# HumaticsLAB/SEAM-Match-RCNN

Measured on AMD Instinct MI355X. Metric: video-clips/sec (10f x 800^2, 32 ROI/f, 1k gallery), higher is better.
Workload: dtype f32; 1 GPU; configs[1] full pipeline, fixed ROIs: 10 frames 800x800 -> ResNet-50-FPN + RPN head -> RoIAlign 14x14 (32 ROI/frame) -> mask head -> match trunk x2 -> SEAM NLB + attention pool (32 seq x 10) -> pair logits vs 1000-product bank -> top-20; hip_graph=False, hip_streams=2, frames=10, rois_per_frame=32, gallery=1000, topk=20, parallelism=single GPU

## Files before the change

include/seam_hip.h:

```cpp
#ifndef SEAM_HIP_H
#define SEAM_HIP_H

#include <stdint.h>

#ifdef __cplusplus
extern "C" {
#endif

typedef void* seam_stream_t;

int seam_version(void);
int seam_fastdiv_exact(unsigned d, unsigned long long n_max);
const char* seam_error_string(int code);

int seam_option_count(void);
const char* seam_option_name(int index);
int seam_set_option(const char* name, int value);
int seam_get_option(const char* name, int* value);

int seam_conv_kred(int C, int R, int S);
int seam_conv_rows_padded(int K);
int seam_conv_tile(int M, int K);
int seam_conv_tile_prec(int prec, int M, int K);
int seam_conv_tile_taps(int prec, int M, int K, int taps);
// ... 19 lines not shown

int seam_conv2d_dual_f32(const float* x1, const float* x2, const float* w_packed, const float* scale,
                         const float* shift, float* y, int N, int Ho, int Wo, int C1, int H2, int W2, int C2,
                         int stride2, int K, int relu, seam_stream_t stream);

int seam_conv1x1_sw_config(int M, int C1, int C2, int K);
int seam_conv1x1_sw_f32(const float* x, const float* x2, const float* w, const float* shift, const float* residual, float* y,
                        int M, int C1, int C2, int K, int relu, int res_mode, int Ho, int Wo, int rH, int rW,
                        seam_stream_t stream);

int seam_conv1x1_f16pc_supported(long long M, int C, int K);
long long seam_conv1x1_f16pc_weight_halves(int K, int C);
int seam_pack_conv1x1_weight_f16pc(const float* w, void* w_packed, int K, int C, seam_stream_t stream);
int seam_conv1x1_f16pc(const void* x, const void* w_packed, const float* scale, const float* shift, const void* residual, void* y,
                       long long M, int C, int K, int relu, seam_stream_t stream);

int seam_conv1x1_swh_config(long long M, int C1, int C2, int K);
int seam_conv1x1_swh_f16(const void* x, const void* x2, const void* w, const float* scale, const float* shift,
                         const void* residual, void* y, long long M, int C1, int C2, int K, int relu, int res_mode,
                         int Ho, int Wo, int rH, int rW, seam_stream_t stream);

int seam_stem_s2d_swh_f16(const void* xpad, const void* w, const float* scale, const float* shift, void* y, int N, int Ho, int Wo,
                          int relu, seam_stream_t stream);

int seam_conv1x1_pc_supported(long long M, int C, int K);
long long seam_conv1x1_pc_weight_floats(int K, int C);
int seam_pack_conv1x1_pc_f32(const float* w, float* w_packed, int K, int C, seam_stream_t stream);
int seam_conv1x1_pc_f32(const float* x, const float* w_packed, const float* scale, const float* shift, const float* residual,
                        float* y, long long M, int C, int K, int relu, seam_stream_t stream);

// ... 305 lines not shown
                             int64_t ws_bytes, const int64_t* scan, int* positions, int64_t capacity, int n, seam_stream_t stream);
int seam_rle_positions_paste(int D, int H, int W, const void* ws, int64_t ws_bytes, const int64_t* scan, int* positions,
                             int64_t capacity, seam_stream_t stream);

#define SEAM_SGD_MAX_SLOTS 32
#define SEAM_SGD_FP_SLOTS 64
typedef struct { float* p; const float* g; float* buf; int64_t numel; int group; int reserved; } seam_sgd_tensor_t;
typedef struct { int tensor; int count; int64_t offset; } seam_sgd_chunk_t;
typedef struct { float lr, momentum, one_minus_dampening, weight_decay; int nesterov, maximize, first, reserved; } seam_sgd_group_t;
typedef struct { int n; int reserved[3]; seam_sgd_group_t g[SEAM_SGD_MAX_SLOTS]; } seam_sgd_groups_t;
int seam_sgd_chunk_elems(void);
int seam_sgd_step_f32(const seam_sgd_tensor_t* tensors, const seam_sgd_chunk_t* chunks, int n_chunks,
                      const seam_sgd_groups_t* groups, unsigned long long* fingerprint, seam_stream_t stream);

enum { SEAM_REPACK_IGEMM = 0, SEAM_REPACK_WINO = 1, SEAM_REPACK_WINO24 = 2, SEAM_REPACK_PC = 3, SEAM_REPACK_SW = 4,
       SEAM_REPACK_SPLIT3 = 5, SEAM_REPACK_NARROW = 6 };
typedef struct {
    const float* src; void* dst; const float* scale;
    int64_t items;
    int form, K, Cin, R, S, Cstore, mode;
    int kred, rows, first_block, n_blocks, reserved;
} seam_repack_job_t;
long long seam_repack_layout(seam_repack_job_t* jobs, int n_jobs);
int seam_repack_many_f32(const seam_repack_job_t* jobs, int n_jobs, long long total_blocks, seam_stream_t stream);

#ifdef __cplusplus
}
#endif
#endif
```

seam-match-rcnn_amd/_native.py:

```python
from __future__ import annotations

import ctypes as C
import os

import torch

_HERE = os.path.dirname(os.path.abspath(__file__))
LIB_PATH = os.environ.get("SEAM_LIB_PATH") or os.path.join(_HERE, "lib", "libseam_hip.so")

_p = C.c_void_p
_i = C.c_int
_f = C.c_float
_i64 = C.c_int64

class TrunkLayer(C.Structure):
    _fields_ = [("w", C.c_void_p), ("u", C.c_void_p), ("u24", C.c_void_p), ("scale", C.c_void_p), ("shift", C.c_void_p)]


SGD_MAX_SLOTS = 32
SGD_FP_SLOTS = 64


class SgdTensor(C.Structure):
    _fields_ = [("p", C.c_void_p), ("g", C.c_void_p), ("buf", C.c_void_p), ("numel", C.c_int64), ("group", C.c_int), ("reserved", C.c_int)]


class SgdChunk(C.Structure):
    _fields_ = [("tensor", C.c_int), ("count", C.c_int), ("offset", C.c_int64)]


class SgdGroup(C.Structure):
    _fields_ = [("lr", C.c_float), ("momentum", C.c_float), ("one_minus_dampening", C.c_float), ("weight_decay", C.c_float),
                ("nesterov", C.c_int), ("maximize", C.c_int), ("first", C.c_int), ("reserved", C.c_int)]


class SgdGroups(C.Structure):
    _fields_ = [("n", C.c_int), ("reserved", C.c_int * 3), ("g", SgdGroup * SGD_MAX_SLOTS)]


REPACK_IGEMM, REPACK_WINO, REPACK_WINO24, REPACK_PC, REPACK_SW, REPACK_SPLIT3, REPACK_NARROW = range(7)


class RepackJob(C.Structure):
    _fields_ = [("src", C.c_void_p), ("dst", C.c_void_p), ("scale", C.c_void_p), ("items", C.c_int64),
                ("form", C.c_int), ("K", C.c_int), ("Cin", C.c_int), ("R", C.c_int), ("S", C.c_int), ("Cstore", C.c_int), ("mode", C.c_int),
                ("kred", C.c_int), ("rows", C.c_int), ("first_block", C.c_int), ("n_blocks", C.c_int), ("reserved", C.c_int)]


SIGNATURES = {
    "seam_version": (_i, []),
    "seam_fastdiv_exact": (_i, [C.c_uint, C.c_ulonglong]),
    "seam_error_string": (C.c_char_p, [_i]),
    "seam_option_count": (_i, []),
    "seam_option_name": (C.c_char_p, [_i]),
    "seam_set_option": (_i, [C.c_char_p, _i]),
# ... 13 lines not shown
    "seam_preprocess_s2d_batch_f32": (_i, [_p, C.c_size_t, _p, _i, _i, _i, _i, _i, _i, _i, _p]),
    "seam_preprocess_s2d_batch_f16": (_i, [_p, C.c_size_t, _p, _i, _i, _i, _i, _i, _i, _i, _p]),
    "seam_preprocess_s2d_pad_batch_f16": (_i, [_p, C.c_size_t, _p, _i, _i, _i, _i, _i, _i, _i, _i, _i, _p]),
    "seam_conv2d_dual_f32": (_i, [_p, _p, _p, _p, _p, _p, _i, _i, _i, _i, _i, _i, _i, _i, _i, _i, _p]),
    "seam_conv1x1_pc_supported": (_i, [C.c_longlong, _i, _i]),
    "seam_conv1x1_pc_weight_floats": (C.c_longlong, [_i, _i]),
    "seam_pack_conv1x1_pc_f32": (_i, [_p, _p, _i, _i, _p]),
    "seam_conv1x1_pc_f32": (_i, [_p, _p, _p, _p, _p, _p, C.c_longlong, _i, _i, _i, _p]),
    "seam_conv1x1_sw_config": (_i, [_i, _i, _i, _i]),
    "seam_conv1x1_sw_f32": (_i, [_p, _p, _p, _p, _p, _p, _i, _i, _i, _i, _i, _i, _i, _i, _i, _i, _p]),
    "seam_conv1x1_swh_config": (_i, [C.c_longlong, _i, _i, _i]),
    "seam_conv1x1_f16pc_supported": (_i, [C.c_longlong, _i, _i]),
    "seam_conv1x1_f16pc_weight_halves": (C.c_longlong, [_i, _i]),
    "seam_pack_conv1x1_weight_f16pc": (_i, [_p, _p, _i, _i, _p]),
    "seam_conv1x1_f16pc": (_i, [_p, _p, _p, _p, _p, _p, C.c_longlong, _i, _i, _i, _p]),
    "seam_conv1x1_swh_f16": (_i, [_p, _p, _p, _p, _p, _p, _p, C.c_longlong, _i, _i, _i, _i, _i, _i, _i, _i, _i, _p]),
    "seam_stem_s2d_swh_f16": (_i, [_p, _p, _p, _p, _p, _i, _i, _i, _i, _p]),
    "seam_conv2d_dual_f16": (_i, [_p, _p, _p, _p, _p, _p, _i, _i, _i, _i, _i, _i, _i, _i, _i, _i, _p]),
    "seam_conv2d_upres_f32": (_i, [_p, _p, _p, _p, _p, _p, _i, _i, _i, _i, _i, _i, _i, _i, _i, _i, _i, _i, _p]),
    "seam_pack_conv_weight_bx3": (_i, [_p, _p, _p, _i, _i, _i, _i, _i, _i, _p]),
    "seam_conv2d_bx3": (_i, [_p, _p, _p, _p, _p, _p, _i, _i, _i, _i, _i, _i, _i, _i, _i, _i, _p]),
    "seam_pack_conv_weight_sx": (_i, [_p, _p, _p, _i, _i, _i, _i, _i, _i, _p]),
    "seam_conv2d_sx": (_i, [_p, _p, _p, _p, _p, _p, _i, _i, _i, _i, _i, _i, _i, _i, _i, _i, _i, _p]),
    "seam_wino_supported": (_i, [_i, _i, _i, _i, _i]),
    "seam_wino_weight_floats": (C.c_longlong, [_i, _i]),
    "seam_wino_slot_fill_pct": (_i, [_i, _i, _i, _i, _i, _i]),
    "seam_wino_tile_variant": (_i, [_i, _i, _i, _i, _i, _i]),
    "seam_pack_conv_weight_wino_f32": (_i, [_p, _p, _i, _i, _i, _i, _p]),
    "seam_wino_issue_slots": (C.c_longlong, [_i, _i, _i, _i, _i, _i]),
    "seam_wino24_issue_slots": (C.c_longlong, [_i, _i, _i, _i, _i, _i]),
# ... 177 lines not shown
```

seam-match-rcnn_amd/csrc/seam_conv.hip:

```cpp
#include <hip/hip_runtime.h>
#include "seam_device.h"
#include "seam_launch.h"
#include <stdint.h>
#include <stdio.h>
#include <stdlib.h>
#include "seam_fastdiv.h"
#include "seam_fpn_common.h"
#include "seam_opts.h"
#include "seam_pack_items.h"

namespace {

constexpr int CHUNK_BYTES = 128;
constexpr int LDB = CHUNK_BYTES + 16;

struct ConvArgs {
    const void* x;
    const void* w;
    const float* scale;
    const float* shift;
    const void* res;
    void* y;
    int N, H, W, C;
    int Ho, Wo, K;
// ... 706 lines not shown
                eo[r] = (unsigned)(row * p.K + n);
            }
            if (p.res) {
#pragma unroll
                for (int r = 0; r < 16; ++r)
                    rv[r] = __builtin_bit_cast(float, __builtin_amdgcn_raw_buffer_load_b32(r_rsrc, nok ? eo[r] * 4u : kOob, 0, 0));
            }
#pragma unroll
            for (int r = 0; r < 16; ++r) {
                float v = acc[i][j][r] * sc + sh;
                if (p.res) v = p.relu == 2 ? (rv[r] > 0.f ? v : 0.f) : v + rv[r];
                if (p.relu == 1) v = fmaxf(v, 0.f);
                __builtin_amdgcn_raw_buffer_store_b32(__builtin_bit_cast(unsigned, v), y_rsrc, nok ? eo[r] * 4u : kOob, 0, 0);
            }
        }
    }
}

__device__ __forceinline__ float top16(float x) {
    unsigned t = __builtin_bit_cast(unsigned, x) & 0xffff0000u;
    asm volatile("" : "+v"(t));
    return __builtin_bit_cast(float, t);
}

__device__ __forceinline__ void split3_bf16(const f32x4 v, u32x2& p0, u32x2& p1, u32x2& p2) {
#pragma unroll
    for (int p = 0; p < 2; ++p) {
        const float a0 = top16(v[2 * p]), b0 = top16(v[2 * p + 1]);
        const float ra = v[2 * p] - a0, rb = v[2 * p + 1] - b0;
        const float a1 = top16(ra), b1 = top16(rb);
        const float sa = ra - a1, sb = rb - b1;
        p0[p] = (__builtin_bit_cast(unsigned, a0) >> 16) | __builtin_bit_cast(unsigned, b0);
        p1[p] = (__builtin_bit_cast(unsigned, a1) >> 16) | __builtin_bit_cast(unsigned, b1);
        p2[p] = (__builtin_bit_cast(unsigned, sa) >> 16) | (__builtin_bit_cast(unsigned, sb) & 0xffff0000u);
    }
}

template <int BM, int BN, int TERMS>
__global__ __launch_bounds__(256, BM * BN >= 128 * 128 ? 1 : 2) void conv_igemm_sx(const ConvArgs p) {
    static_assert(TERMS == 6 || TERMS == 9, "six or nine piece products");
    constexpr int NW = 4, ES = 4, EPV = 4, BKE = 32;
    constexpr int WM = BM / 2, WN = BN / 2;
    constexpr int MT = WM / 32, NT = WN / 32;
    constexpr int RP = 8 * NW;
    constexpr int AI = BM / RP;
    constexpr int VPP = BN * 4;
    constexpr int BI = 3 * VPP / 256;
    constexpr int Q = TERMS * MT * NT;
    constexpr int PA = BM * 64 + 64;
// ... 617 lines not shown
```

seam-match-rcnn_amd/csrc/seam_pack_items.h:

```cpp
#pragma once
#include <hip/hip_runtime.h>
#include <stddef.h>
#include "seam_device.h"

namespace seam_pack {

template <int BKE>
__device__ __forceinline__ float igemm_value(const float* __restrict__ w, size_t i, int K, int Cin, int R, int S, int Cstore, int nk,
                                             int bn, int mode) {
    const int col = (int)(i % BKE);
    size_t rest = i / BKE;
    const int row_in = (int)(rest % bn);
    rest /= bn;
    const int q = (int)(rest % nk);
    const int tn = (int)(rest / nk);
    const int row = tn * bn + row_in;
    int r, s2, c;
    if (Cstore >= BKE) {
        const int ccn = Cstore / BKE;
        s2 = q % S;
        c = ((q / S) % ccn) * BKE + col;
        r = q / (S * ccn);
    } else {
        const int kk = q * BKE + col;
// ... 105 lines not shown
        }
    }
}

__device__ __forceinline__ void pwpc_item(const float* __restrict__ w, float* __restrict__ out, size_t i, int C) {
    const int nsteps = C / 8;
    const int lane = (int)(i & 63);
    size_t rest = i >> 6;
    const int step = (int)(rest % nsteps); rest /= nsteps;
    const int nt = (int)rest;
    const int nn = nt * 32 + (lane & 31);
    const int c = 8 * step + 4 * (lane >> 5);
    *reinterpret_cast<f32x4*>(out + i * 4) = *reinterpret_cast<const f32x4*>(w + (size_t)nn * C + c);
}

__device__ __forceinline__ void narrow_item(const float* __restrict__ w, float* __restrict__ out, int i, int K, int C) {
    const int e = i & 3, lane = (i >> 2) & 63, j = i >> 8;
    const int col = lane & 15, kq = lane >> 4;
    out[i] = col < K ? w[(size_t)col * C + 16 * j + 4 * kq + e] : 0.f;
}

__device__ __forceinline__ void sw_item(const float* __restrict__ w, const float* __restrict__ scale, float* __restrict__ out, size_t i, int C) {
    const float v = w[i];
    out[i] = scale ? v * scale[i / (size_t)C] : v;
}

}
```

seam-match-rcnn_amd/csrc/seam_repack.hip:

```cpp
#include <hip/hip_runtime.h>
#include <stdint.h>
#include "seam_device.h"
#include "seam_hip.h"
#include "seam_pack_items.h"

namespace {

constexpr int JOB_BLOCKS = 512;

__global__ __launch_bounds__(256) void repack_many_kernel(const seam_repack_job_t* __restrict__ jobs, int n_jobs) {
    int lo = 0, hi = n_jobs;
    while (hi - lo > 1) {
        const int mid = lo + ((hi - lo) >> 1);
        if (jobs[mid].first_block <= (int)blockIdx.x) lo = mid; else hi = mid;
    }
    const seam_repack_job_t j = jobs[lo];
    const size_t i0 = (size_t)((int)blockIdx.x - j.first_block) * 256 + threadIdx.x;
    const size_t step = (size_t)j.n_blocks * 256;
    const size_t total = (size_t)j.items;
    const float* src = j.src;
    switch (j.form) {
    case SEAM_REPACK_IGEMM: {
        const int nk = j.kred / 32, bn = j.rows % 128 == 0 ? 128 : 64;
        float* out = (float*)j.dst;
// ... 4 lines not shown
        const int nk = j.kred / 32, bn = j.rows % 128 == 0 ? 128 : 64;
        unsigned short* out = (unsigned short*)j.dst;
        for (size_t i = i0; i < total; i += step)
            seam_pack::split3_item(seam_pack::igemm_value<32>(src, i, j.K, j.Cin, j.R, j.S, j.Cstore, nk, bn, j.mode), out, i, bn);
        break;
    }
    case SEAM_REPACK_WINO:
        for (size_t i = i0; i < total; i += step) seam_pack::wino_item(src, (float*)j.dst, i, j.K, j.Cin, j.Cstore / 8, j.mode);
        break;
    case SEAM_REPACK_WINO24:
        for (size_t i = i0; i < total; i += step) seam_pack::wino24_item(src, (float*)j.dst, i, j.K, j.Cin, j.Cstore / 8, j.mode);
        break;
    case SEAM_REPACK_PC:
        for (size_t i = i0; i < total; i += step) seam_pack::pwpc_item(src, (float*)j.dst, i, j.Cstore);
        break;
    case SEAM_REPACK_SW:
        for (size_t i = i0; i < total; i += step) seam_pack::sw_item(src, j.scale, (float*)j.dst, i, j.Cstore);
        break;
    case SEAM_REPACK_NARROW:
        for (size_t i = i0; i < total; i += step) seam_pack::narrow_item(src, (float*)j.dst, (int)i, j.K, j.Cstore);
        break;
    default:
        break;
    }
}

long long job_items(seam_repack_job_t& j) {
    if (!j.src || !j.dst || j.K < 1 || j.Cin < 1 || j.Cstore < j.Cin) return 0;
    const bool one = j.R == 1 && j.S == 1, plain = j.Cstore == j.Cin && j.mode == 0 && one;
    switch (j.form) {
// ... 2 lines not shown
        if (j.R < 1 || j.S < 1 || (j.Cstore % 4) || (j.Cstore >= 32 && j.Cstore % 32) || j.mode < 0 || j.mode > 2) return 0;
        if (j.mode == 1 && (!one || j.K % 4)) return 0;
        if ((long long)j.R * j.S * j.Cstore > (1 << 24)) return 0;
        j.kred = seam_conv_kred(j.Cstore, j.R, j.S);
        j.rows = seam_conv_rows_padded(j.K);
        return (long long)j.rows * j.kred;
    }
    case SEAM_REPACK_WINO:
    case SEAM_REPACK_WINO24:
        if (j.R != 3 || j.S != 3 || (j.mode != 0 && j.mode != 2) || !seam_wino_supported(j.Cstore, j.K, 3, 3, 1)) return 0;
        if ((j.K % 32) || (j.Cstore % 8)) return 0;
        return (long long)(j.K / 32) * (j.Cstore / 8) * 64;
    case SEAM_REPACK_PC:
        if (!plain || (j.K % 128) || (j.Cstore % 128) || (((uintptr_t)j.src | (uintptr_t)j.dst) & 15)) return 0;
        return (long long)j.K * j.Cstore / 4;
    case SEAM_REPACK_SW:
        if (!plain) return 0;
        return (long long)j.K * j.Cstore;
    case SEAM_REPACK_NARROW:
        if (!plain || !seam_linear_narrow_supported(j.Cstore, j.K)) return 0;
        return (long long)(j.Cstore >> 4) * 256;
    default:
        return 0;
    }
}

}

extern "C" {

// ... 28 lines not shown
```

seam-match-rcnn_amd/ops.py:

```python
from __future__ import annotations

import ctypes as C
from dataclasses import dataclass
from typing import Optional, Sequence

import torch

from . import _native

F32 = torch.float32
F16 = torch.float16


def _stream() -> int:
    return torch.cuda.current_stream().cuda_stream


def _req(t: torch.Tensor, dtype=F32, name: str = "tensor") -> torch.Tensor:
    if not isinstance(t, torch.Tensor) or not t.is_cuda:
        raise _native.SeamNativeError(f"{name}: expected a tensor on the HIP device (no CPU path exists)")
    if dtype is not None and t.dtype != dtype:
        raise TypeError(f"{name}: expected {dtype}, got {t.dtype}")
    return t if t.is_contiguous() else t.contiguous()

# ... 19 lines not shown
    R: int
    S: int
    stride: int = 1
    pad: int = 0
    Cin: int = 0
    dtype: object = F32
    u: Optional[torch.Tensor] = None
    u24: Optional[torch.Tensor] = None
    wn: Optional[torch.Tensor] = None
    ws: Optional[torch.Tensor] = None
    shift_sw: Optional[torch.Tensor] = None
    wq: Optional[torch.Tensor] = None
    wh: Optional[torch.Tensor] = None
    wsh: Optional[torch.Tensor] = None
    wph: Optional[torch.Tensor] = None


BX3 = "bf16x3"
SX6 = "bf16x6"
SX9 = "bf16x9"
_SX_TERMS = {SX6: 6, SX9: 9}


import os as _os
WINOGRAD = _os.environ.get("SEAM_WINOGRAD", "1") != "0"
F16PC = _os.environ.get("SEAM_F16PC", "1") != "0"
F16PC64 = _os.environ.get("SEAM_F16PC64", "1") != "0"
PWPC = _os.environ.get("SEAM_PWPC", "1") != "0"
SWH = _os.environ.get("SEAM_PWH", "1") != "0"
PWHPC = _os.environ.get("SEAM_PWHPC", "1") != "0"
PWHPC_MIN_C = int(_os.environ.get("SEAM_PWHPC_MIN_C", "1024"))
F16PC_RULE = True


def _pack_wino(lib, weight: torch.Tensor, K: int, cin: int, cs: int, mode: int) -> Optional[torch.Tensor]:
    if not lib.seam_wino_supported(cs, K, 3, 3, 1):
        return None
    u = torch.empty((int(lib.seam_wino_weight_floats(K, cs)),), dtype=F32, device=weight.device)
    _native.check(lib.seam_pack_conv_weight_wino_f32(_ptr(weight), _ptr(u), K, cin, cs, mode, _stream()),
                  "seam_pack_conv_weight_wino_f32")
    return u


def _pack_wino24(lib, weight: torch.Tensor, K: int, cin: int, cs: int, mode: int) -> Optional[torch.Tensor]:
    if not lib.seam_wino_supported(cs, K, 3, 3, 1):
        return None
# ... 70 lines not shown
    if transposed2x2:
        cin, cout = weight.shape[0], weight.shape[1]
        K, R, S, mode = 4 * cout, 1, 1, 1
    else:
        is_linear = weight.dim() == 2
        if weight.dim() == 2:
            weight = weight[:, :, None, None]
        if weight.dim() == 3:
            weight = weight[:, :, :, None]
        weight = weight.contiguous()
        K, cin, R, S = weight.shape
        mode = 0
    epv = 8 if dtype == F16 else 4
    cs = cstore if cstore is not None else ((cin + epv - 1) // epv) * epv
    rows = lib.seam_conv_rows_padded(K)
    u = u24 = wh = None
    if dtype == F32:
        kred = lib.seam_conv_kred(cs, R, S)
        wp = torch.empty((rows, kred), dtype=F32, device=weight.device)
        _native.check(lib.seam_pack_conv_weight_f32(_ptr(weight), _ptr(wp), K, cin, R, S, cs, mode, _stream()),
                      "seam_pack_conv_weight_f32")
        if wino and mode == 0 and R == 3 and S == 3 and stride == 1:
            u = _pack_wino(lib, weight, K, cin, cs, 0)
            u24 = _pack_wino24(lib, weight, K, cin, cs, 0) if u is not None else None
    elif dtype == BX3:
        kred = lib.seam_conv_kred(cs, R, S)
        wp = torch.empty((rows, kred), dtype=F32, device=weight.device)
        tmp = torch.empty((rows, kred), dtype=F32, device=weight.device)
        _native.check(lib.seam_pack_conv_weight_bx3(_ptr(weight), _ptr(wp), _ptr(tmp), K, cin, R, S, cs, mode, _stream()),
                      "seam_pack_conv_weight_bx3")
    elif dtype in _SX_TERMS:
        kred = lib.seam_conv_kred(cs, R, S)
        wp = torch.empty((rows, kred * 3), dtype=torch.bfloat16, device=weight.device)
        tmp = torch.empty((rows, kred), dtype=F32, device=weight.device)
        _native.check(lib.seam_pack_conv_weight_sx(_ptr(weight), _ptr(wp), _ptr(tmp), K, cin, R, S, cs, mode, _stream()),
                      "seam_pack_conv_weight_sx")
    else:
        kred = lib.seam_conv_kred_f16(cs, R, S)
        wp = torch.empty((rows, kred), dtype=F16, device=weight.device)
        _native.check(lib.seam_pack_conv_weight_f16(_ptr(weight), _ptr(wp), K, cin, R, S, cs, mode, _stream()),
                      "seam_pack_conv_weight_f16")
        if F16PC and mode == 0 and R == 3 and S == 3 and stride == 1 and pad in (0, 1) and ((cs % 128 == 0 and K % 128 == 0) or (cs == 64 and K == 64 and F16PC64)):
            wh = torch.empty((int(lib.seam_f16pc_weight_halves(K, cs)),), dtype=F16, device=weight.device)
            _native.check(lib.seam_pack_conv_weight_f16pc(_ptr(weight), _ptr(wh), K, cin, cs, _stream()), "seam_pack_conv_weight_f16pc")
    scale = shift = None
    if bias is not None:
        bias = bias.detach().to(F32)
        if transposed2x2:
            bias = bias.repeat(4)
    if bn is not None:
        bw, bb, rm, rv = (t.detach().to(F32) for t in bn)
# ... 20 lines not shown
            and lib.seam_conv1x1_pc_supported(1 << 20, cs, K)):
        wq = torch.empty((int(lib.seam_conv1x1_pc_weight_floats(K, cs)),), dtype=F32, device=weight.device)
        _native.check(lib.seam_pack_conv1x1_pc_f32(_ptr(weight.reshape(K, cin).to(F32).contiguous()), _ptr(wq), K, cs, _stream()),
                      "seam_pack_conv1x1_pc_f32")
    wsh = None
    if (SWH and dtype == F16 and mode in (0, 1) and not is_linear and R == 1 and S == 1 and stride == 1 and pad == 0 and cs == cin
            and lib.seam_conv1x1_swh_config(1 << 20, cs, 0, K)):
        wm = weight.permute(2, 3, 1, 0).reshape(K, cin) if transposed2x2 else weight.reshape(K, cin)
        wsh = wm.to(F16).contiguous()
    wph = None
    if (PWHPC and dtype == F16 and mode == 0 and not is_linear and R == 1 and S == 1 and stride == 1 and pad == 0 and cs == cin
            and lib.seam_conv1x1_f16pc_supported(1 << 20, cs, K)):
        wph = torch.empty((int(lib.seam_conv1x1_f16pc_weight_halves(K, cs)),), dtype=F16, device=weight.device)
        _native.check(lib.seam_pack_conv1x1_weight_f16pc(_ptr(weight.reshape(K, cin).to(F32).contiguous()), _ptr(wph), K, cs, _stream()),
                      "seam_pack_conv1x1_weight_f16pc")
    pc = PackedConv(wp, scale, shift, K, cs, R, S, stride, pad, cin, dtype, u, u24, wn, ws, shift_sw, wq, wh, wsh, wph)
    if _PACK_RECORDER is not None:
        _PACK_RECORDER.records.append((weight, bias, bn, mode, pc))
    return pc


def pack_conv_dgrad(weight: torch.Tensor, pad_fwd: int = 0, wino: bool = True) -> PackedConv:
    lib = _native.lib()
    weight = _req(weight.detach(), name="weight")
    if weight.dim() == 2:
        weight = weight[:, :, None, None]
    weight = weight.contiguous()
    cout, cin, R, S = weight.shape
    if cout % 32 or R != S:
        raise ValueError("pack_conv_dgrad: Cout must be a multiple of 32 and the kernel square")
    rows = lib.seam_conv_rows_padded(cin)
# ... 181 lines not shown
        e0, e1 = torch.cuda.Event(enable_timing=True), torch.cuda.Event(enable_timing=True)
        e0.record()
    lib = _native.lib()
    wino = pc.dtype == F32 and pc.u is not None and WINOGRAD and out_hw is None and _wino_pays(lib, n, h, w, c, pc.K, pc.pad)
    wino24 = wino and pc.u24 is not None and WINOGRAD24 and _wino24_pays(lib, n, h, w, c, pc.K, pc.pad)
    sw = not narrow and pc.dtype == F32 and out_hw is None and _sw_ok(pc, h, w)
    pwpc = (not narrow and not sw and pc.dtype == F32 and pc.wq is not None and PWPC and out_hw is None and h * w >= PWPC_MIN_HW
            and lib.seam_conv1x1_pc_supported(n * h * w, c, pc.K) == 1)
    f16pc = (pc.dtype == F16 and pc.wh is not None and F16PC and residual is None and out_hw is None and not out_f32 and relu in (0, 1, False, True)
             and (lib.seam_conv3x3_f16pc_pays if F16PC_RULE else lib.seam_conv3x3_f16pc_supported)(n, h, w, c, pc.K, pc.pad) == 1)
    pwhpc = (pc.dtype == F16 and pc.wph is not None and PWHPC and residual is None and out_hw is None and not out_f32
             and relu in (0, 1, False, True) and c >= PWHPC_MIN_C and h * w >= SW_MIN_HW
             and lib.seam_conv1x1_f16pc_supported(n * h * w, c, pc.K) == 1)
    swh = (not pwhpc and pc.dtype == F16 and pc.wsh is not None and SWH and out_hw is None and not out_f32 and h * w >= SW_MIN_HW
           and relu in (0, 1, False, True))
    if pwhpc:
        _native.check(lib.seam_conv1x1_f16pc(_ptr(x), _ptr(pc.wph), _ptr(pc.scale), _ptr(pc.shift), None, _ptr(y), n * h * w, c, pc.K,
                                             1 if relu else 0, _stream()), "seam_conv1x1_f16pc")
    elif swh:
        _native.check(lib.seam_conv1x1_swh_f16(_ptr(x), None, _ptr(pc.wsh), _ptr(pc.scale), _ptr(pc.shift), _ptr(residual), _ptr(y),
                                               n * h * w, c, 0, pc.K, 1 if relu else 0, 1 if residual is not None else 0, 0, 0, 0, 0,
                                               _stream()), "seam_conv1x1_swh_f16")
    elif narrow:
        _native.check(lib.seam_linear_narrow_f32(_ptr(x), _ptr(pc.wn), _ptr(pc.shift), _ptr(y), n * h * w, c, pc.K, int(relu), _stream()),
                      "seam_linear_narrow_f32")
    elif sw:
        _sw_launch(lib, x, None, pc, residual, y, n * h * w, c, 0, relu, 1 if residual is not None else 0)
    elif pwpc:
        _native.check(lib.seam_conv1x1_pc_f32(_ptr(x), _ptr(pc.wq), _ptr(pc.scale), _ptr(pc.shift), _ptr(residual), _ptr(y),
                                              n * h * w, c, pc.K, int(relu), _stream()), "seam_conv1x1_pc_f32")
    elif wino24:
# ... 17 lines not shown
    elif pc.dtype == BX3:
        _native.check(lib.seam_conv2d_bx3(_ptr(x), _ptr(pc.w), _ptr(pc.scale), _ptr(pc.shift), _ptr(residual), _ptr(y),
                                          n, h, w, c, pc.K, pc.R, pc.S, pc.stride, pc.pad, int(relu), _stream()),
                      "seam_conv2d_bx3")
    elif f16pc:
        _native.check(lib.seam_conv3x3_f16pc(_ptr(x), _ptr(pc.wh), _ptr(pc.scale), _ptr(pc.shift), None, _ptr(y),
                                             n, h, w, c, pc.K, pc.pad, 1 if relu else 0, _stream()), "seam_conv3x3_f16pc")
    else:
        _native.check(lib.seam_conv2d_f16(_ptr(x), _ptr(pc.w), _ptr(pc.scale), _ptr(pc.shift), _ptr(residual), _ptr(y),
                                          n, h, w, c, pc.K, pc.R, pc.S, pc.stride, pc.pad, 1 if relu else 0,
                                          1 if out_f32 else 0, _stream()), "seam_conv2d_f16")
    if trace is not None:
        e1.record()
        tile = lib.seam_conv_tile_taps(3 if pc.dtype in _SX_TERMS else 2 if pc.dtype == BX3 else 1 if pc.dtype == F16 else 0,
                                       n * ho * wo, pc.K, pc.R * pc.S)
        if pwhpc:
            variant = "conv1x1_f16pc"
        elif swh:
            variant = _swh_variant(lib, n * h * w, c, pc.K)
        elif narrow:
            variant = "linear_narrow"
        elif sw:
            variant = _sw_variant(lib, n * h * w, c, pc.K)
        elif pwpc:
            variant = "conv1x1_pc"
        elif wino24:
            variant = ("conv3x3_wino24pc" if lib.seam_wino24_form(n, h, w, c, pc.K, pc.pad) == 1
                       else f"conv3x3_wino24<{lib.seam_wino24_variant(n, h, w, c, pc.K, pc.pad)}>")
        elif wino:
            variant = f"conv3x3_wino<{lib.seam_wino_tile_variant(n, h, w, c, pc.K, pc.pad)}>"
        elif f16pc:
# ... 1382 lines not shown
                self._entries.append((wdeps, self._jobs_of(path, weight, mode, pc)))
            self._pk.append(pk)
            self._keys.append(m._pack_key())
        self.rebuilds += self._ever_built
        self._built = self._ever_built = True

    @staticmethod
    def _jobs_of(path, weight, mode, pc):
        N = _native

        def job(form, dst, R=1, S=1, cs=pc.Cstore, cin=pc.Cin, md=0, scale=None):
            return N.RepackJob(src=weight.data_ptr(), dst=dst.data_ptr(), scale=None if scale is None else scale.data_ptr(), form=form,
                               K=pc.K, Cin=cin, R=R, S=S, Cstore=cs, mode=md)

        if pc.dtype in _SX_TERMS:
            return [job(N.REPACK_SPLIT3, pc.w, pc.R, pc.S, md=mode)]
        if pc.dtype != F32 or pc.wh is not None or pc.wsh is not None or pc.wph is not None:
            raise NotImplementedError(f"PackPlan: {path}: only fp32 packs are refreshed in place (pass refresh_packs=False)")
        jobs = [job(N.REPACK_IGEMM, pc.w, pc.R, pc.S, md=mode)]
        if pc.u is not None:
            jobs.append(job(N.REPACK_WINO, pc.u, 3, 3, md=mode))
        if pc.u24 is not None:
            jobs.append(job(N.REPACK_WINO24, pc.u24, 3, 3, md=mode))
        if (pc.wn is not None or pc.ws is not None or pc.wq is not None) and mode != 0:
            raise NotImplementedError(f"PackPlan: {path}: the pointwise forms of a transposed conv are not covered")
        if pc.wn is not None:
            jobs.append(job(N.REPACK_NARROW, pc.wn))
        if pc.ws is not None and pc.ws.data_ptr() != weight.data_ptr():
            jobs.append(job(N.REPACK_SW, pc.ws, scale=pc.scale))
        if pc.wq is not None:
            jobs.append(job(N.REPACK_PC, pc.wq))
# ... 52 lines not shown
```

Before: 69.68 clips/s.

## Add warp-specialized persistent split-bf16 MFMA kernel for large SX6 1x1 convs

Adds a new persistent 1x1 convolution kernel for SX6 (bf16x3 split, six-term) packed layers. Producer waves load fp32 activations, split them into three bf16 planes in LDS, and double-buffer them. Consumer waves run 32x32x16 bf16 MFMAs against a pre-split weight pack streamed through a register ring, then apply a fused scale/shift/residual/relu epilogue. The kernel is used only when the tile count passes a threshold, and it adds a third weight pack per eligible layer plus a repack path. The aim is to replace the generic SX implicit-GEMM kernel for large pointwise convs with better overlap of loads and compute.

```diff
diff --git a/include/seam_hip.h b/include/seam_hip.h
--- a/include/seam_hip.h
+++ b/include/seam_hip.h
@@ -57,6 +57,12 @@
 int seam_pack_conv1x1_weight_f16pc(const float* w, void* w_packed, int K, int C, seam_stream_t stream);
 int seam_conv1x1_f16pc(const void* x, const void* w_packed, const float* scale, const float* shift, const void* residual, void* y,
                        long long M, int C, int K, int relu, seam_stream_t stream);
+
+int seam_conv1x1_sxpc_supported(long long M, int C, int K);
+long long seam_conv1x1_sxpc_weight_bytes(int K, int C);
+int seam_pack_conv1x1_weight_sxpc(const float* w, void* w_packed, int K, int C, seam_stream_t stream);
+int seam_conv1x1_sxpc(const float* x, const void* w_packed, const float* scale, const float* shift, const float* residual, float* y,
+                      long long M, int C, int K, int relu, seam_stream_t stream);
 
 int seam_conv1x1_swh_config(long long M, int C1, int C2, int K);
 int seam_conv1x1_swh_f16(const void* x, const void* x2, const void* w, const float* scale, const float* shift,
@@ -392,7 +398,7 @@
                       const seam_sgd_groups_t* groups, unsigned long long* fingerprint, seam_stream_t stream);
 
 enum { SEAM_REPACK_IGEMM = 0, SEAM_REPACK_WINO = 1, SEAM_REPACK_WINO24 = 2, SEAM_REPACK_PC = 3, SEAM_REPACK_SW = 4,
-       SEAM_REPACK_SPLIT3 = 5, SEAM_REPACK_NARROW = 6 };
+       SEAM_REPACK_SPLIT3 = 5, SEAM_REPACK_NARROW = 6, SEAM_REPACK_SXPC = 7 };
 typedef struct {
     const float* src; void* dst; const float* scale;
     int64_t items;
diff --git a/seam-match-rcnn_amd/_native.py b/seam-match-rcnn_amd/_native.py
--- a/seam-match-rcnn_amd/_native.py
+++ b/seam-match-rcnn_amd/_native.py
@@ -38,7 +38,7 @@
     _fields_ = [("n", C.c_int), ("reserved", C.c_int * 3), ("g", SgdGroup * SGD_MAX_SLOTS)]
 
 
-REPACK_IGEMM, REPACK_WINO, REPACK_WINO24, REPACK_PC, REPACK_SW, REPACK_SPLIT3, REPACK_NARROW = range(7)
+REPACK_IGEMM, REPACK_WINO, REPACK_WINO24, REPACK_PC, REPACK_SW, REPACK_SPLIT3, REPACK_NARROW, REPACK_SXPC = range(8)
 
 
 class RepackJob(C.Structure):
@@ -82,6 +82,10 @@
     "seam_conv1x1_f16pc_weight_halves": (C.c_longlong, [_i, _i]),
     "seam_pack_conv1x1_weight_f16pc": (_i, [_p, _p, _i, _i, _p]),
     "seam_conv1x1_f16pc": (_i, [_p, _p, _p, _p, _p, _p, C.c_longlong, _i, _i, _i, _p]),
+    "seam_conv1x1_sxpc_supported": (_i, [C.c_longlong, _i, _i]),
+    "seam_conv1x1_sxpc_weight_bytes": (C.c_longlong, [_i, _i]),
+    "seam_pack_conv1x1_weight_sxpc": (_i, [_p, _p, _i, _i, _p]),
+    "seam_conv1x1_sxpc": (_i, [_p, _p, _p, _p, _p, _p, C.c_longlong, _i, _i, _i, _p]),
     "seam_conv1x1_swh_f16": (_i, [_p, _p, _p, _p, _p, _p, _p, C.c_longlong, _i, _i, _i, _i, _i, _i, _i, _i, _i, _p]),
     "seam_stem_s2d_swh_f16": (_i, [_p, _p, _p, _p, _p, _i, _i, _i, _i, _p]),
     "seam_conv2d_dual_f16": (_i, [_p, _p, _p, _p, _p, _p, _i, _i, _i, _i, _i, _i, _i, _i, _i, _i, _p]),
diff --git a/seam-match-rcnn_amd/csrc/seam_conv.hip b/seam-match-rcnn_amd/csrc/seam_conv.hip
--- a/seam-match-rcnn_amd/csrc/seam_conv.hip
+++ b/seam-match-rcnn_amd/csrc/seam_conv.hip
@@ -744,25 +744,6 @@
                 __builtin_amdgcn_raw_buffer_store_b32(__builtin_bit_cast(unsigned, v), y_rsrc, nok ? eo[r] * 4u : kOob, 0, 0);
             }
         }
-    }
-}
-
-__device__ __forceinline__ float top16(float x) {
-    unsigned t = __builtin_bit_cast(unsigned, x) & 0xffff0000u;
-    asm volatile("" : "+v"(t));
-    return __builtin_bit_cast(float, t);
-}
-
-__device__ __forceinline__ void split3_bf16(const f32x4 v, u32x2& p0, u32x2& p1, u32x2& p2) {
-#pragma unroll
-    for (int p = 0; p < 2; ++p) {
-        const float a0 = top16(v[2 * p]), b0 = top16(v[2 * p + 1]);
-        const float ra = v[2 * p] - a0, rb = v[2 * p + 1] - b0;
-        const float a1 = top16(ra), b1 = top16(rb);
-        const float sa = ra - a1, sb = rb - b1;
-        p0[p] = (__builtin_bit_cast(unsigned, a0) >> 16) | __builtin_bit_cast(unsigned, b0);
-        p1[p] = (__builtin_bit_cast(unsigned, a1) >> 16) | __builtin_bit_cast(unsigned, b1);
-        p2[p] = (__builtin_bit_cast(unsigned, sa) >> 16) | (__builtin_bit_cast(unsigned, sb) & 0xffff0000u);
     }
 }
 
diff --git a/seam-match-rcnn_amd/csrc/seam_pack_items.h b/seam-match-rcnn_amd/csrc/seam_pack_items.h
--- a/seam-match-rcnn_amd/csrc/seam_pack_items.h
+++ b/seam-match-rcnn_amd/csrc/seam_pack_items.h
@@ -2,6 +2,7 @@
 #include <hip/hip_runtime.h>
 #include <stddef.h>
 #include "seam_device.h"
+#include "seam_split.h"
 
 namespace seam_pack {
 
@@ -143,6 +144,27 @@
     *reinterpret_cast<f32x4*>(out + i * 4) = *reinterpret_cast<const f32x4*>(w + (size_t)nn * C + c);
 }
 
+__device__ __forceinline__ void sxpc_item(const float* __restrict__ w, unsigned short* __restrict__ out, size_t i, int C) {
+    const int nsteps = C / 16;
+    const int lane = (int)(i & 63);
+    const size_t rest = i >> 6;
+    const int step = (int)(rest % nsteps);
+    const size_t nt = rest / nsteps;
+    const float* src = w + (nt * 32 + (lane & 31)) * (size_t)C + 16 * step + 8 * (lane >> 5);
+    unsigned short* o = out + (nt * nsteps + step) * 1536 + lane * 8;
+#pragma unroll
+    for (int e = 0; e < 8; ++e) {
+        const float x = src[e];
+        const float x0 = top16(x);
+        const float r = x - x0;
+        const float y0 = top16(r);
+        const float s = r - y0;
+        o[e] = (unsigned short)(__builtin_bit_cast(unsigned, x0) >> 16);
+        o[512 + e] = (unsigned short)(__builtin_bit_cast(unsigned, y0) >> 16);
+        o[1024 + e] = (unsigned short)(__builtin_bit_cast(unsigned, s) >> 16);
+    }
+}
+
 __device__ __forceinline__ void narrow_item(const float* __restrict__ w, float* __restrict__ out, int i, int K, int C) {
     const int e = i & 3, lane = (i >> 2) & 63, j = i >> 8;
     const int col = lane & 15, kq = lane >> 4;
diff --git a/seam-match-rcnn_amd/csrc/seam_pwsx.hip b/seam-match-rcnn_amd/csrc/seam_pwsx.hip
--- /dev/null
+++ b/seam-match-rcnn_amd/csrc/seam_pwsx.hip
@@ -0,0 +1,325 @@
+#include <hip/hip_runtime.h>
+#include "seam_device.h"
+#include <stdint.h>
+#include <type_traits>
+#include "seam_fastdiv.h"
+#include "seam_launch.h"
+#include "seam_pack_items.h"
+#include "seam_split.h"
+
+namespace {
+
+constexpr int BM = 128;
+constexpr int CK = 64;
+constexpr int KS = CK / 16;
+constexpr int PLB = CK * 2;
+constexpr int ROWB = 3 * PLB + 16;
+constexpr int ABUF = BM * ROWB;
+constexpr int NP = BM * (CK / 4) / 256;
+constexpr int TROW = 128 + 16;
+constexpr int TBUF = 32 * TROW;
+constexpr int TR0 = 2 * ABUF;
+constexpr int LDS_BYTES = TR0 + 4 * 2 * TBUF;
+static_assert(LDS_BYTES <= 160 * 1024 && ABUF + 3 * PLB < 65536 && 4 * 32 * ROWB < 65536, "LDS map / ds immediates");
+constexpr int RB = 4;
+static_assert(RB == KS, "ring slot = k-step of the chunk");
+constexpr int RVA = 3;
+
+#ifndef SEAM_SXPC_ABL
+#define SEAM_SXPC_ABL 0
+#endif
+
+struct SxpcArgs {
+    const float* x;
+    const void* w;
+    const float* scale;
+    const float* shift;
+    const float* res;
+    float* y;
+    int M, C, K, relu;
+    int tiles_n, nchunks, total_tiles;
+    unsigned m_tiles_n;
+};
+
+__global__ __launch_bounds__(512, 2) void conv1x1_sxpc(const SxpcArgs p) {
+    extern __shared__ __attribute__((aligned(16))) char smem[];
+    const int tid = threadIdx.x, lane = tid & 63;
+    const int wave = __builtin_amdgcn_readfirstlane(tid >> 6);
+    const bool consumer = wave < 4;
+    const int n = p.nchunks;
+
+    const XcdTiles xt = xcd_tiles(p.total_tiles);
+    const int ntiles = xt.ntiles, S = xt.stride;
+    if (ntiles == 0) return;
+    const int tile0 = xt.tile0();
+    const size_t row_bytes = (size_t)p.C * 4, out_row = (size_t)p.K * 4;
+    const int total_chunks = ntiles * n;
+
+    if (!consumer) {
+        const int ptid = tid - 256;
+        unsigned goff[NP];
+        LDSQ char* lp[NP];
+#pragma unroll
+        for (int r = 0; r < NP; ++r) {
+            const int row = (ptid >> 4) + 16 * r;
+            goff[r] = (unsigned)(row * p.C * 4 + (ptid & 15) * 16);
+            lp[r] = (LDSQ char*)smem + row * ROWB + (ptid & 15) * 8;
+        }
+        f32x4 rq[2][NP];
+        int tile = tile0, ck = 0, tiles_left = ntiles;
+        auto x_desc = [&](const int tl) {
+            const int tm = fdivu(tl, p.tiles_n, p.m_tiles_n);
+            const int row0 = tm * BM;
+            const int rows = tiles_left > 0 ? min(BM, p.M - row0) : 0;
+            return __builtin_amdgcn_make_buffer_rsrc((void*)((const char*)p.x + (size_t)(tiles_left > 0 ? row0 : 0) * row_bytes), 0,
+                                                     (int)(rows * row_bytes), 0x00020000);
+        };
+        __amdgpu_buffer_rsrc_t rs = x_desc(tile);
+        auto request = [&](f32x4 (&dst)[NP]) {
+#pragma unroll
+            for (int r = 0; r < NP; ++r)
+                dst[r] = __builtin_bit_cast(f32x4, __builtin_amdgcn_raw_buffer_load_b128(rs, (SEAM_SXPC_ABL & 1) ? kOob : goff[r], ck * (CK * 4), 0));
+            if (++ck == n) {
+                ck = 0;
+                tile += S;
+                --tiles_left;
+                rs = x_desc(tile);
+            }
+        };
+        auto store_chunk = [&](const f32x4 (&src)[NP], const int buf) {
+            if (SEAM_SXPC_ABL & 1) return;
+#pragma unroll
+            for (int r = 0; r < NP; ++r) {
+                u32x2 q0, q1, q2;
+                if (SEAM_SXPC_ABL & 4) {
+                    q0[0] = __builtin_bit_cast(unsigned, src[r][0]); q0[1] = __builtin_bit_cast(unsigned, src[r][1]);
+                    q1[0] = __builtin_bit_cast(unsigned, src[r][2]); q1[1] = __builtin_bit_cast(unsigned, src[r][3]); q2 = q0;
+                } else {
+                    split3_bf16(src[r], q0, q1, q2);
+                }
+                *reinterpret_cast<u32x2 LDSQ*>(lp[r] + buf * ABUF) = q0;
+                *reinterpret_cast<u32x2 LDSQ*>(lp[r] + buf * ABUF + PLB) = q1;
+                *reinterpret_cast<u32x2 LDSQ*>(lp[r] + buf * ABUF + 2 * PLB) = q2;
+            }
+        };
+        request(rq[0]);
+        request(rq[1]);
+        store_chunk(rq[0], 0);
+        request(rq[0]);
+        LDS_BAR();
+        for (int c = 0; c < total_chunks; c += 2) {
+            store_chunk(rq[1], 1);
+            request(rq[1]);
+            LDS_BAR();
+            if (c + 1 >= total_chunks) break;
+            store_chunk(rq[0], 0);
+            request(rq[0]);
+            LDS_BAR();
+        }
+    } else {
+        const int wn = wave;
+        f32x16 acc[4];
+        f32x4 af[3][4];
+        f32x4 bf[RB][3];
+        const LDSQ char* ac = (const LDSQ char*)smem + (lane & 31) * ROWB + (lane >> 5) * 16;
+        const LDSQ char* an = ac + ABUF;
+        const int nsteps = p.C >> 4;
+        const int wtile_bytes = nsteps * 3072;
+        const int blane = lane * 16;
+        __amdgpu_buffer_rsrc_t w_rsrc;
+        int tm_n = 0, tn_n = 0;
+        auto load_b = [&](const int slot, const int step) {
+#pragma unroll
+            for (int pl = 0; pl < 3; ++pl)
+                bf[slot][pl] = __builtin_bit_cast(f32x4, __builtin_amdgcn_raw_buffer_load_b128(w_rsrc, blane, (step * 3 + pl) * 1024, 0));
+        };
+        auto ring_preload = [&](const int tl) {
+            tm_n = fdivu(tl, p.tiles_n, p.m_tiles_n);
+            tn_n = __builtin_amdgcn_readfirstlane(tl - tm_n * p.tiles_n);
+            tm_n = __builtin_amdgcn_readfirstlane(tm_n);
+            w_rsrc = __builtin_amdgcn_make_buffer_rsrc((void*)((const char*)p.w + (size_t)(tn_n * 4 + wn) * wtile_bytes), 0, wtile_bytes, 0x00020000);
+#pragma unroll
+            for (int s = 0; s < RB; ++s) { SB(); load_b(s, s); }
+            SB();
+        };
+        const unsigned ooff = (unsigned)((lane >> 3) * p.K * 4 + (32 * wn + 4 * (lane & 7)) * 4);
+        LDSQ char* const tw = (LDSQ char*)smem + TR0 + wn * (2 * TBUF) + (lane & 31) * TROW + (lane >> 5) * 16;
+        const LDSQ char* const tr = (const LDSQ char*)smem + TR0 + wn * (2 * TBUF) + (lane >> 3) * TROW + (lane & 7) * 16;
+        const int K32 = 32 * p.K * 4, K8 = 8 * p.K * 4;
+        int tile = tile0;
+        ring_preload(tile);
+        f32x4 rv[4][4], sc, sh;
+        LDS_BAR();
+        for (int k = 0; k < ntiles; ++k) {
+            const int tm_k = tm_n, tn_k = tn_n;
+            const int rows = min(BM, p.M - tm_k * BM);
+            const __amdgpu_buffer_rsrc_t y_rsrc = __builtin_amdgcn_make_buffer_rsrc(
+                (void*)((char*)p.y + (size_t)tm_k * BM * out_row), 0, (int)(rows * out_row), 0x00020000);
+            const __amdgpu_buffer_rsrc_t r_rsrc = __builtin_amdgcn_make_buffer_rsrc(
+                (void*)((const char*)(p.res ? p.res : p.y) + (size_t)tm_k * BM * out_row), 0, (int)(rows * out_row), 0x00020000);
+            const unsigned ocol = ooff + (unsigned)(tn_k * 512);
+#pragma unroll
+            for (int pl = 0; pl < 3; ++pl)
+#pragma unroll
+                for (int m = 0; m < 4; ++m) af[pl][m] = *reinterpret_cast<const f32x4 LDSQ*>(ac + m * (32 * ROWB) + pl * PLB);
+            for (int t = 0; t < n; ++t) {
+                const bool last = t == n - 1;
+                if (last) {
+                    const int ch = tn_k * 128 + 32 * wn + 4 * (lane & 7);
+                    const f32x4 a = *reinterpret_cast<const f32x4*>((p.scale ? p.scale : (const float*)p.w) + ch);
+                    const f32x4 b = *reinterpret_cast<const f32x4*>((p.shift ? p.shift : (const float*)p.w) + ch);
+                    sc = a;
+                    sh = b;
+                    if (p.res) {
+#pragma unroll
+                        for (int m = 0; m < RVA; ++m)
+#pragma unroll
+                            for (int i = 0; i < 4; ++i)
+                                rv[m][i] = __builtin_bit_cast(f32x4, __builtin_amdgcn_raw_buffer_load_b128(r_rsrc, ocol + m * K32 + i * K8, 0, 0));
+                    }
+                }
+                auto read_a = [&](const int pl, const int m, const int ks) -> f32x4 {
+                    return *reinterpret_cast<const f32x4 LDSQ*>((ks == KS ? an : ac + ks * 32) + m * (32 * ROWB) + pl * PLB);
+                };
+#pragma unroll
+                for (int ks = 0; ks < KS; ++ks) {
+                    constexpr int TA[6] = {2, 1, 0, 1, 0, 0}, TB[6] = {0, 1, 2, 0, 1, 0};
+                    constexpr int LAST[3] = {5, 3, 0};
+#pragma unroll
+                    for (int tq = 0; tq < 6; ++tq) {
+                        const int pa = TA[tq], pb = TB[tq];
+                        if (ks == KS - 1 && tq == 1) {
+                            SB();
+                            LDS_BAR();
+                            SB();
+#if !(SEAM_SXPC_ABL & 8)
+#pragma unroll
+                            for (int m = 0; m < 4; ++m) af[2][m] = read_a(2, m, KS);
+#endif
+                        }
+#pragma unroll
+                        for (int m = 0; m < 4; ++m) {
+                            SB();
+                            if (ks == 0 && tq == 0 && t == 0) {
+                                const f32x16 z = {0.f, 0.f, 0.f, 0.f, 0.f, 0.f, 0.f, 0.f, 0.f, 0.f, 0.f, 0.f, 0.f, 0.f, 0.f, 0.f};
+                                acc[m] = __builtin_amdgcn_mfma_f32_32x32x16_bf16(__builtin_bit_cast(bf16x8, bf[ks][pb]), __builtin_bit_cast(bf16x8, af[pa][m]), z, 0, 0, 0);
+                            } else {
+                                acc[m] = __builtin_amdgcn_mfma_f32_32x32x16_bf16(__builtin_bit_cast(bf16x8, bf[ks][pb]), __builtin_bit_cast(bf16x8, af[pa][m]), acc[m], 0, 0, 0);
+                            }
+                            SB();
+#if !(SEAM_SXPC_ABL & 8)
+                            if (tq == LAST[pa] && !(ks == KS - 1 && tq == 0)) af[pa][m] = read_a(pa, m, ks + 1);
+#endif
+                        }
+                    }
+                    SB();
+#if !(SEAM_SXPC_ABL & 2)
+                    load_b(ks, min(t * KS + ks + RB, nsteps - 1));
+#endif
+                }
+                SB();
+                const LDSQ char* const sw = ac;
+                ac = an;
+                an = sw;
+            }
+            tile += S;
+            ring_preload(tile);
+            if (!p.scale) sc = f32x4{1.f, 1.f, 1.f, 1.f};
+            if (!p.shift) sh = f32x4{0.f, 0.f, 0.f, 0.f};
+            auto finish_tile = [&](auto res_c, auto relu_c) {
+                constexpr bool RES = decltype(res_c)::value, RELU = decltype(relu_c)::value;
+                if (RES) {
+#pragma unroll
+                    for (int m = RVA; m < 4; ++m)
+#pragma unroll
+                        for (int i = 0; i < 4; ++i)
+                            rv[m][i] = __builtin_bit_cast(f32x4, __builtin_amdgcn_raw_buffer_load_b128(r_rsrc, ocol + m * K32 + i * K8, 0, 0));
+#pragma unroll
+                    for (int m = 0; m < 4; ++m) asm volatile("" :: "v"(rv[m][0]), "v"(rv[m][1]), "v"(rv[m][2]), "v"(rv[m][3]));
+                }
+                auto put = [&](const int m) {
+#pragma unroll
+                    for (int qd = 0; qd < 4; ++qd)
+                        *reinterpret_cast<f32x4 LDSQ*>(tw + (m & 1) * TBUF + qd * 32) =
+                            f32x4{acc[m][4 * qd], acc[m][4 * qd + 1], acc[m][4 * qd + 2], acc[m][4 * qd + 3]};
+                };
+                put(0);
+#pragma unroll
+                for (int m = 0; m < 4; ++m) {
+                    if (m + 1 < 4) put(m + 1);
+#pragma unroll
+                    for (int i = 0; i < 4; ++i) {
+                        f32x4 v = *reinterpret_cast<const f32x4 LDSQ*>(tr + (m & 1) * TBUF + i * (8 * TROW));
+                        v = v * sc + sh;
+                        if (RES) v += rv[m][i];
+                        if (RELU) {
+#pragma unroll
+                            for (int e = 0; e < 4; ++e) v[e] = fmaxf(v[e], 0.f);
+                        }
+                        __builtin_amdgcn_raw_buffer_store_b128(__builtin_bit_cast(u32x4, v), y_rsrc, ocol + m * K32 + i * K8, 0, 0);
+                    }
+                }
+            };
+            if (p.res) {
+                if (p.relu) finish_tile(std::true_type{}, std::true_type{}); else finish_tile(std::true_type{}, std::false_type{});
+            } else {
+                if (p.relu) finish_tile(std::false_type{}, std::true_type{}); else finish_tile(std::false_type{}, std::false_type{});
+            }
+        }
+    }
+}
+
+__global__ void sxpc_pack_kernel(const float* __restrict__ w, unsigned short* __restrict__ out, int K, int C) {
+    const size_t total = (size_t)K * C / 8;
+    for (size_t i = (size_t)blockIdx.x * blockDim.x + threadIdx.x; i < total; i += (size_t)gridDim.x * blockDim.x)
+        seam_pack::sxpc_item(w, out, i, C);
+}
+
+int sxpc_plan(SxpcArgs& a, long long M, int C, int K) {
+    if (M <= 0 || C < 256 || (C % CK) || K < 128 || (K % 128)) return 1;
+    if ((unsigned long long)BM * C * 4 >= kOob || (unsigned long long)BM * K * 4 >= kOob) return 1;
+    if ((unsigned long long)(C / 16) * 3072 >= kOob) return 1;
+    const long long tiles_m = (M + BM - 1) / BM;
+    const long long total = tiles_m * (K / 128);
+    if (total >= (1LL << 24) || M >= (1LL << 31)) return 1;
+    a.M = (int)M; a.C = C; a.K = K;
+    a.tiles_n = K / 128; a.nchunks = C / CK; a.total_tiles = (int)total;
+    if (!seam_fastdiv::exact(a.tiles_n, 2ull * total + (1ull << 16))) return 1;
+    a.m_tiles_n = seam_fastdiv::magic(a.tiles_n);
+    return 0;
+}
+
+}
+
+extern "C" {
+
+int seam_conv1x1_sxpc_supported(long long M, int C, int K) {
+    SxpcArgs a;
+    return sxpc_plan(a, M, C, K) == 0 ? 1 : 0;
+}
+
+long long seam_conv1x1_sxpc_weight_bytes(int K, int C) { return (long long)K * C * 6; }
+
+int seam_pack_conv1x1_weight_sxpc(const float* w, void* w_packed, int K, int C, void* stream) {
+    SxpcArgs a;
+    if (sxpc_plan(a, 1, C, K)) return (int)hipErrorInvalidValue;
+    const size_t total = (size_t)K * C / 8;
+    const unsigned grid = seam_launch::grid256(total);
+    hipLaunchKernelGGL(sxpc_pack_kernel, dim3(grid), dim3(256), 0, (hipStream_t)stream, w, (unsigned short*)w_packed, K, C);
+    return (int)hipGetLastError();
+}
+
+int seam_conv1x1_sxpc(const float* x, const void* w_packed, const float* scale, const float* shift, const float* residual, float* y,
+                      long long M, int C, int K, int relu, void* stream) {
+    SxpcArgs a;
+    if ((relu != 0 && relu != 1) || sxpc_plan(a, M, C, K)) return (int)hipErrorInvalidValue;
+    a.x = x; a.w = w_packed; a.scale = scale; a.shift = shift; a.res = residual; a.y = y; a.relu = relu;
+    int ncu;
+    const hipError_t e = seam_launch::prepare<conv1x1_sxpc>(LDS_BYTES, &ncu);
+    if (e != hipSuccess) return (int)e;
+    const unsigned grid = (unsigned)(a.total_tiles > ncu ? ncu : a.total_tiles);
+    hipLaunchKernelGGL(conv1x1_sxpc, dim3(grid), dim3(512), LDS_BYTES, (hipStream_t)stream, a);
+    return (int)hipGetLastError();
+}
+
+}
diff --git a/seam-match-rcnn_amd/csrc/seam_repack.hip b/seam-match-rcnn_amd/csrc/seam_repack.hip
--- a/seam-match-rcnn_amd/csrc/seam_repack.hip
+++ b/seam-match-rcnn_amd/csrc/seam_repack.hip
@@ -42,6 +42,9 @@
     case SEAM_REPACK_PC:
         for (size_t i = i0; i < total; i += step) seam_pack::pwpc_item(src, (float*)j.dst, i, j.Cstore);
         break;
+    case SEAM_REPACK_SXPC:
+        for (size_t i = i0; i < total; i += step) seam_pack::sxpc_item(src, (unsigned short*)j.dst, i, j.Cstore);
+        break;
     case SEAM_REPACK_SW:
         for (size_t i = i0; i < total; i += step) seam_pack::sw_item(src, j.scale, (float*)j.dst, i, j.Cstore);
         break;
@@ -74,6 +77,9 @@
     case SEAM_REPACK_PC:
         if (!plain || (j.K % 128) || (j.Cstore % 128) || (((uintptr_t)j.src | (uintptr_t)j.dst) & 15)) return 0;
         return (long long)j.K * j.Cstore / 4;
+    case SEAM_REPACK_SXPC:
+        if (!plain || !seam_conv1x1_sxpc_supported(1, j.Cstore, j.K)) return 0;
+        return (long long)j.K * j.Cstore / 8;
     case SEAM_REPACK_SW:
         if (!plain) return 0;
         return (long long)j.K * j.Cstore;
diff --git a/seam-match-rcnn_amd/csrc/seam_split.h b/seam-match-rcnn_amd/csrc/seam_split.h
--- /dev/null
+++ b/seam-match-rcnn_amd/csrc/seam_split.h
@@ -0,0 +1,22 @@
+#pragma once
+#include <hip/hip_runtime.h>
+#include "seam_device.h"
+
+__device__ __forceinline__ float top16(float x) {
+    unsigned t = __builtin_bit_cast(unsigned, x) & 0xffff0000u;
+    asm volatile("" : "+v"(t));
+    return __builtin_bit_cast(float, t);
+}
+
+__device__ __forceinline__ void split3_bf16(const f32x4 v, u32x2& p0, u32x2& p1, u32x2& p2) {
+#pragma unroll
+    for (int p = 0; p < 2; ++p) {
+        const float a0 = top16(v[2 * p]), b0 = top16(v[2 * p + 1]);
+        const float ra = v[2 * p] - a0, rb = v[2 * p + 1] - b0;
+        const float a1 = top16(ra), b1 = top16(rb);
+        const float sa = ra - a1, sb = rb - b1;
+        p0[p] = (__builtin_bit_cast(unsigned, a0) >> 16) | __builtin_bit_cast(unsigned, b0);
+        p1[p] = (__builtin_bit_cast(unsigned, a1) >> 16) | __builtin_bit_cast(unsigned, b1);
+        p2[p] = (__builtin_bit_cast(unsigned, sa) >> 16) | (__builtin_bit_cast(unsigned, sb) & 0xffff0000u);
+    }
+}
diff --git a/seam-match-rcnn_amd/ops.py b/seam-match-rcnn_amd/ops.py
--- a/seam-match-rcnn_amd/ops.py
+++ b/seam-match-rcnn_amd/ops.py
@@ -57,6 +57,7 @@
     wh: Optional[torch.Tensor] = None
     wsh: Optional[torch.Tensor] = None
     wph: Optional[torch.Tensor] = None
+    wx: Optional[torch.Tensor] = None
 
 
 BX3 = "bf16x3"
@@ -73,6 +74,9 @@
 SWH = _os.environ.get("SEAM_PWH", "1") != "0"
 PWHPC = _os.environ.get("SEAM_PWHPC", "1") != "0"
 PWHPC_MIN_C = int(_os.environ.get("SEAM_PWHPC_MIN_C", "1024"))
+SXPC = _os.environ.get("SEAM_SXPC", "1") != "0"
+SXPC_MIN_TILES = int(_os.environ.get("SEAM_SXPC_MIN_TILES", "196"))
+SXPC_RULE = True
 F16PC_RULE = True
 
 
@@ -173,7 +177,7 @@
     epv = 8 if dtype == F16 else 4
     cs = cstore if cstore is not None else ((cin + epv - 1) // epv) * epv
     rows = lib.seam_conv_rows_padded(K)
-    u = u24 = wh = None
+    u = u24 = wh = wx = None
     if dtype == F32:
         kred = lib.seam_conv_kred(cs, R, S)
         wp = torch.empty((rows, kred), dtype=F32, device=weight.device)
@@ -194,6 +198,11 @@
         tmp = torch.empty((rows, kred), dtype=F32, device=weight.device)
         _native.check(lib.seam_pack_conv_weight_sx(_ptr(weight), _ptr(wp), _ptr(tmp), K, cin, R, S, cs, mode, _stream()),
                       "seam_pack_conv_weight_sx")
+        if (SXPC and dtype == SX6 and mode == 0 and not is_linear and R == 1 and S == 1 and stride == 1 and pad == 0 and cs == cin
+                and lib.seam_conv1x1_sxpc_supported(1 << 20, cs, K)):
+            wx = torch.empty((int(lib.seam_conv1x1_sxpc_weight_bytes(K, cs)),), dtype=torch.uint8, device=weight.device)
+            _native.check(lib.seam_pack_conv1x1_weight_sxpc(_ptr(weight.reshape(K, cin).to(F32).contiguous()), _ptr(wx), K, cs, _stream()),
+                          "seam_pack_conv1x1_weight_sxpc")
     else:
         kred = lib.seam_conv_kred_f16(cs, R, S)
         wp = torch.empty((rows, kred), dtype=F16, device=weight.device)
@@ -244,7 +253,7 @@
         wph = torch.empty((int(lib.seam_conv1x1_f16pc_weight_halves(K, cs)),), dtype=F16, device=weight.device)
         _native.check(lib.seam_pack_conv1x1_weight_f16pc(_ptr(weight.reshape(K, cin).to(F32).contiguous()), _ptr(wph), K, cs, _stream()),
                       "seam_pack_conv1x1_weight_f16pc")
-    pc = PackedConv(wp, scale, shift, K, cs, R, S, stride, pad, cin, dtype, u, u24, wn, ws, shift_sw, wq, wh, wsh, wph)
+    pc = PackedConv(wp, scale, shift, K, cs, R, S, stride, pad, cin, dtype, u, u24, wn, ws, shift_sw, wq, wh, wsh, wph, wx)
     if _PACK_RECORDER is not None:
         _PACK_RECORDER.records.append((weight, bias, bn, mode, pc))
     return pc
@@ -456,7 +465,12 @@
              and lib.seam_conv1x1_f16pc_supported(n * h * w, c, pc.K) == 1)
     swh = (not pwhpc and pc.dtype == F16 and pc.wsh is not None and SWH and out_hw is None and not out_f32 and h * w >= SW_MIN_HW
            and relu in (0, 1, False, True))
-    if pwhpc:
+    sxpc = (pc.dtype == SX6 and pc.wx is not None and SXPC and out_hw is None and relu in (0, 1, False, True)
+            and (-(-(n * h * w) // 128) * (pc.K // 128) >= SXPC_MIN_TILES or not SXPC_RULE) and lib.seam_conv1x1_sxpc_supported(n * h * w, c, pc.K) == 1)
+    if sxpc:
+        _native.check(lib.seam_conv1x1_sxpc(_ptr(x), _ptr(pc.wx), _ptr(pc.scale), _ptr(pc.shift), _ptr(residual), _ptr(y), n * h * w, c, pc.K,
+                                            1 if relu else 0, _stream()), "seam_conv1x1_sxpc")
+    elif pwhpc:
         _native.check(lib.seam_conv1x1_f16pc(_ptr(x), _ptr(pc.wph), _ptr(pc.scale), _ptr(pc.shift), None, _ptr(y), n * h * w, c, pc.K,
                                              1 if relu else 0, _stream()), "seam_conv1x1_f16pc")
     elif swh:
@@ -504,7 +518,9 @@
         e1.record()
         tile = lib.seam_conv_tile_taps(3 if pc.dtype in _SX_TERMS else 2 if pc.dtype == BX3 else 1 if pc.dtype == F16 else 0,
                                        n * ho * wo, pc.K, pc.R * pc.S)
-        if pwhpc:
+        if sxpc:
+            variant = "conv1x1_sxpc"
+        elif pwhpc:
             variant = "conv1x1_f16pc"
         elif swh:
             variant = _swh_variant(lib, n * h * w, c, pc.K)
@@ -1917,7 +1933,10 @@
                                K=pc.K, Cin=cin, R=R, S=S, Cstore=cs, mode=md)
 
         if pc.dtype in _SX_TERMS:
-            return [job(N.REPACK_SPLIT3, pc.w, pc.R, pc.S, md=mode)]
+            jobs = [job(N.REPACK_SPLIT3, pc.w, pc.R, pc.S, md=mode)]
+            if pc.wx is not None:
+                jobs.append(job(N.REPACK_SXPC, pc.wx))
+            return jobs
         if pc.dtype != F32 or pc.wh is not None or pc.wsh is not None or pc.wph is not None:
             raise NotImplementedError(f"PackPlan: {path}: only fp32 packs are refreshed in place (pass refresh_packs=False)")
         jobs = [job(N.REPACK_IGEMM, pc.w, pc.R, pc.S, md=mode)]
```

After: 71.20 clips/s, median of 6. +2.2%, better.
